# rlorenzo/facet

Measured on AMD Instinct MI355X. Metric: images/sec whole-node (TOPIQ+SAMP+CLIP+InsightFace ensemble), 1024² batch, higher is better.
Workload: dtype f32

## Files before the change

### facet_amd/_lib.py

```python
import ctypes as C
import importlib.util
import os
import sys
import threading

import numpy as np

_HERE = os.path.dirname(os.path.abspath(__file__))
LIB_PATH = os.environ.get("FACET_AMD_LIB") or os.path.join(_HERE, "libfacet_engine.so")

FE_MODEL_TOPIQ, FE_MODEL_CLIP, FE_MODEL_SAMP, FE_MODEL_U2NETP, FE_MODEL_AESTHETIC, FE_MODEL_VLM = range(6)
FE_RECORD_FLOATS = 789
FE_GRAPH_FACE_DET, FE_GRAPH_FACE_LMK, FE_GRAPH_FACE_REC = 0, 1, 2
FE_FACE_FLOATS = 739
FE_STATS_DOUBLES = 264
FILTERS = {"lanczos": 1, "bilinear": 2, "bicubic": 3}
FE_PRECISION_RES32 = 16
FE_PRECISION_SPLIT3 = 32
PRECISION = {"f32": 0, "fp32": 0, "float32": 0, "bf16": 1, "bfloat16": 1, "f16": 2, "fp16": 2, "float16": 2, "half": 2,
             "bf16+r32": 1 | FE_PRECISION_RES32, "f16+r32": 2 | FE_PRECISION_RES32, "f16x3": 2 | FE_PRECISION_RES32 | FE_PRECISION_SPLIT3}
PRECISION_NAME = {0: "f32", 1: "bf16", 2: "f16", 1 | FE_PRECISION_RES32: "bf16+r32", 2 | FE_PRECISION_RES32: "f16+r32",
                  2 | FE_PRECISION_RES32 | FE_PRECISION_SPLIT3: "f16x3"}
ACT = {"none": 0, None: 0, "relu": 1, "gelu": 2, "sigmoid": 3, "softplus": 5, "quickgelu": 6}
ELEM = {"f32": 0, "bf16": 1, "f16": 2}
# ... 45 lines not shown
    "fe_profile_get": (C.c_int, [C.c_void_p, C.c_int, C.c_char_p, C.c_int, C.POINTER(C.c_double),
                                 C.POINTER(C.c_double), _f32p]),
    "fe_flops_reset": (C.c_int, [C.c_void_p]),
    "fe_flops_get": (C.c_int, [C.c_void_p, C.POINTER(C.c_double)]),
    "fe_flops_get_executed": (C.c_int, [C.c_void_p, C.POINTER(C.c_double)]),
    "fe_flops_get_half": (C.c_int, [C.c_void_p, C.POINTER(C.c_double)]),
    "fe_weights_begin": (C.c_int, [C.c_void_p, C.c_int]),
    "fe_weights_set": (C.c_int, [C.c_void_p, C.c_int, C.c_char_p, _f32p, _i64p, C.c_int]),
    "fe_weights_commit": (C.c_int, [C.c_void_p, C.c_int]),
    "fe_model_unload": (C.c_int, [C.c_void_p, C.c_int]),
    "fe_model_loaded": (C.c_int, [C.c_void_p, C.c_int]),
    "fe_op_conv2d": (C.c_int, [C.c_void_p, _f32p, C.c_int, C.c_int, C.c_int, C.c_int, _f32p, C.c_int, C.c_int,
                               C.c_int, _f32p, _f32p, _f32p, C.c_int, C.c_int, C.c_int, C.c_int, C.c_int, _f32p]),
    "fe_op_gate_rowpool": (C.c_int, [C.c_void_p, _f32p, C.c_int, C.c_int, C.c_int, C.c_int, C.c_int, _f32p, _f32p, C.c_int, _f32p, C.c_int,
                                     C.c_int, C.c_int, C.c_int, _f32p, C.POINTER(C.c_int)]),
    "fe_op_topiq_gate64": (C.c_int, [C.c_void_p, _f32p, C.c_int, C.c_int, C.c_int, _f32p, _f32p, _f32p, _f32p, _f32p, C.c_float,
                                     _f32p, _f32p, C.c_int, C.c_int, _f32p]),
    "fe_op_conv3x3_c64": (C.c_int, [C.c_void_p, _f32p, C.c_int, C.c_int, C.c_int, _f32p, _f32p, _f32p, C.c_int, _f32p, _f32p, _f32p,
                                    _f32p, _f32p]),
    "fe_op_maxpool2d": (C.c_int, [C.c_void_p, _f32p, C.c_int, C.c_int, C.c_int, C.c_int, C.c_int, C.c_int,
                                  C.c_int, C.c_int, _f32p]),
    "fe_op_bilinear": (C.c_int, [C.c_void_p, _f32p, C.c_int, C.c_int, C.c_int, C.c_int, C.c_int, C.c_int, _f32p]),
    "fe_op_adaptive_avgpool": (C.c_int, [C.c_void_p, _f32p, C.c_int, C.c_int, C.c_int, C.c_int, C.c_int, C.c_int,
                                         _f32p]),
    "fe_op_layernorm": (C.c_int, [C.c_void_p, _f32p, C.c_int, C.c_int, _f32p, _f32p, C.c_float, _f32p]),
    "fe_op_plane": (C.c_int, [C.c_void_p, C.c_int, C.c_int, _f32p] + [C.c_int] * 14 + [C.c_float, C.c_float, _f32p]),
    "fe_op_rowpass": (C.c_int, [C.c_void_p, C.c_int, C.c_int, C.c_int, _f32p] + [C.c_int] * 6 + [_f32p, _f32p, C.c_int, C.c_int, C.c_float, C.c_float, _f32p]),
    "fe_op_gemm_skinny": (C.c_int, [C.c_void_p, C.c_int, C.c_int, C.c_int, _f32p, C.c_int, C.c_int, C.c_int, _f32p, C.c_int, C.c_int, _f32p, _f32p, C.c_int,
                                    C.c_int, C.c_float, _f32p]),
    "fe_op_attention": (C.c_int, [C.c_void_p, _f32p, _f32p, _f32p, _f32p, C.c_int, C.c_int, C.c_int, C.c_int, C.c_int, C.c_int, _f32p]),
# ... 389 lines not shown
        xr, xp = _f32(xr)
        weight, wp = _f32(weight)
        cout = weight.shape[0]
        assert weight.shape == (cout, cin)
        bp = None
        if bias is not None:
            bias, bp = _f32(bias)
        gate, gp = _f32(gate)
        assert gate.shape == (n, h, w)
        y = np.empty((n, th, tw, cout), np.float32)
        routed = C.c_int(0)
        self._ck(self.lib.fe_op_gate_rowpool(self.h, xp, n, h, w, cin, ldx, wp, bp, cout, gp, ACT[act], th, tw, int(bool(fused)),
                                             y.ctypes.data_as(_f32p), C.byref(routed)))
        return np.ascontiguousarray(y.transpose(0, 3, 1, 2)), bool(routed.value)

    def topiq_gate64(self, x, w0, b0, w2, b2, w4, b4, wx, bx, wblk_act="gelu", gate_act="gelu"):
        x, xp = _f32(x)
        n, c, h, w = x.shape
        assert c == 64
        arrs = [_f32(a) for a in (w0, b0, w2, b2, w4, wx, bx)]
        y = np.empty((n, 64, h // 16, w // 16), np.float32)
        self._ck(self.lib.fe_op_topiq_gate64(self.h, xp, n, h, w, arrs[0][1], arrs[1][1], arrs[2][1], arrs[3][1], arrs[4][1], C.c_float(float(b4)),
                                             arrs[5][1], arrs[6][1], ACT[wblk_act], ACT[gate_act], y.ctypes.data_as(_f32p)))
        return y

    def conv3x3_c64(self, x, w2, scale2=None, shift2=None, act2="relu", w3=None, scale3=None, shift3=None, res=None):
        x, xp = _f32(x)
        n, c, h, w = x.shape
        assert c == 64
        keep = [_f32(a) if a is not None else (None, None) for a in (w2, scale2, shift2, w3, scale3, shift3, res)]
# ... 1136 lines not shown
```

### facet_amd/csrc/capi_ops.hip

```cpp
#include "capi_internal.h"
#include "fp8_core.h"

template <class E>
static E* hook_up(Ctx& C, const float* src, size_t n, int off = 0) {
  if (!src) return nullptr;
  if constexpr (std::is_same_v<E, float>) {
    float* d = C.arena.array<float>(n + off) + off;
    FE_HIP(hipMemcpyAsync(d, src, n * sizeof(float), hipMemcpyHostToDevice, C.stream));
    return d;
  } else {
    const float* d32 = upload(C, src, n);
    E* d = C.arena.array<E>(n + off) + off;
    launch_convert(d32, d, n, C.stream);
    return d;
  }
}
template <class E>
static E* hook_filled(Ctx& C, size_t n, float fill, int off = 0) {
  const std::vector<float> v(n, fill);
  E* d = hook_up<E>(C, v.data(), n, off);
  FE_HIP(hipStreamSynchronize(C.stream));
  return d;
}
template <class E>
// ... 116 lines not shown
    W.shape = {cout, cin}; W.data.assign(weight, weight + (size_t)cout * cin);
    if (bias) { B.shape = {cout}; B.data.assign(bias, bias + cout); }
    ConvW cw = build_linear_rows(dw, W, bias ? &B : nullptr, 0, cout);
    FE_CHECK(cw.CinPad <= ldx, "fe_op_gate_rowpool: ldx below the packed channel count %d", cw.CinPad);
    Tensor xt = C.arena.tensor(n, h, w, ldx);
    FE_HIP(hipMemcpyAsync(xt.p, x, xt.numel() * sizeof(float), hipMemcpyHostToDevice, C.stream));
    Tensor gt = C.arena.tensor(n, h, w, 1);
    FE_HIP(hipMemcpyAsync(gt.p, gate, gt.numel() * sizeof(float), hipMemcpyHostToDevice, C.stream));
    ConvOpts og; og.act = act; og.gate = &gt;
    int took = 0;
    Tensor pooled = topiq_gate_pool(C, cw, xt.slice(0, cw.CinPad), og, th, tw, fused != 0, &took);
    FE_CHECK(pooled.h == th && pooled.w == tw && pooled.ld == cout, "fe_op_gate_rowpool: unexpected result shape");
    FE_HIP(hipMemcpyAsync(y, pooled.p, pooled.numel() * sizeof(float), hipMemcpyDeviceToHost, C.stream));
    FE_HIP(hipStreamSynchronize(C.stream));
    if (routed) *routed = took;
  });
}

int fe_op_topiq_gate64(fe_ctx* ctx, const float* x, int n, int h, int w, const float* w0, const float* b0, const float* w2, const float* b2,
                       const float* w4, float b4, const float* wx, const float* bx, int wblk_act, int gate_act, float* y) {
  return fe_api(ctx, [&] {
    Ctx& C = ctx->c;
    FE_CHECK(x && w0 && b0 && w2 && b2 && w4 && wx && bx && y && n > 0 && h > 0 && w > 0 && h % 16 == 0 && w % 16 == 0, "bad gate64 arguments");
    FE_CHECK(C.precision == PREC_BF16 || C.precision == PREC_F16, "fe_op_topiq_gate64: the fused gate exists for the 2-byte element types only");
    C.arena.reset();
    DeviceWeights dw;
    dw.prec = C.precision;
    GatedConvW g;
    build_gate64_fragments(dw, g, w0, b0, w2, b2, w4, b4, wx, bx);
    auto run = [&](auto* tag) {
// ... 570 lines not shown
```

### facet_amd/csrc/conv_bf16_kernel.h

```cpp
#pragma once
#include "fe_common.h"
#include <cstdlib>

namespace fe {

typedef float h_f32x16 __attribute__((ext_vector_type(16)));
typedef float h_v4f __attribute__((ext_vector_type(4)));
typedef __attribute__((address_space(3))) void* h_lptr_t;

union H8 {
  h_v4f f;
  uint4 u;
};

template <class E>
__device__ __forceinline__ void h_unpack8(const uint4 u, float v[8]) {
  const E* tag = nullptr;
  fe_unpack2(tag, u.x, v[0], v[1]); fe_unpack2(tag, u.y, v[2], v[3]);
  fe_unpack2(tag, u.z, v[4], v[5]); fe_unpack2(tag, u.w, v[6], v[7]);
}


typedef unsigned h_v2u __attribute__((ext_vector_type(2)));
typedef unsigned h_v4u __attribute__((ext_vector_type(4)));
// ... 632 lines not shown
      const bool cok = col < p.Cout;
      const float sc = (cok && p.scale) ? p.scale[col] : 1.f;
      const float sf = (cok && p.shift) ? p.shift[col] : 0.f;
  #pragma unroll
      for (int i = 0; i < TM; ++i) {
  #pragma unroll
        for (int e = 0; e < 16; ++e) {
          const int row = wm * TM * 32 + i * 32 + (e & 3) + 8 * (e >> 2) + 4 * h;
          const int m = m0 + row;
          if (cok && m < p.M) {
            float v = acc[i][j][e] * sc + sf;
            float rs_ = p.res ? (float)p.res[(size_t)m * p.ldr + col] : 0.f;
            if constexpr (S32) { if (p.res32) rs_ = p.res32[(size_t)m * p.ldr32 + col]; }
            if (!p.res_after_act) v += rs_;
            if constexpr (MODE == 2) v = v > 0.f ? v : v * p.slope[col];
            else v = fe_apply_act(v, p.act);
            if (p.res_after_act) v += rs_;
            if (p.gate) v *= (float)p.gate[(size_t)m * p.ldg + (p.gate_c1 ? 0 : col)];
            if constexpr (S32) {
              if (p.y) stf(&p.y[(size_t)m * p.ldy + col], v);
              if (p.y32) p.y32[(size_t)m * p.ldy32 + col] = v;
            } else {
              stf(&p.y[(size_t)m * p.ldy + col], v);
            }
          }
        }
      }
    }
  
    return;
// ... 47 lines not shown
```

### facet_amd/csrc/engine.h

```cpp
#pragma once
#include "fe_common.h"
#include "../../include/facet_engine.h"
#include <memory>
#include <tuple>

namespace fe {

struct HostTensor {
  std::vector<float> data;
  std::vector<int64_t> shape;
  size_t numel() const { size_t n = 1; for (auto d : shape) n *= (size_t)d; return n; }
};

class WeightStore {
 public:
  void clear() { t_.clear(); }
  void set(const std::string& name, const float* data, const int64_t* shape, int ndim);
  bool has(const std::string& name) const { return t_.count(name) != 0; }
  const HostTensor& get(const std::string& name) const;
  size_t size() const { return t_.size(); }
 private:
  std::map<std::string, HostTensor> t_;
};

// ... 66 lines not shown
  void* wv_h = nullptr;
  float* bv = nullptr;
  ConvW out;
  int d = 0, heads = 0;
};
MHAW build_mha(DeviceWeights& dw, const WeightStore& ws, const std::string& prefix, int heads);
template <class T, class RT>
void mha_forward(Ctx& c, const MHAW& m, const T* q_in, int ldq, const T* kv_in, int ldkv, int B, int Lq,
                 int Lk, const RT* res, int ldr, RT* y, int ldy, bool causal = false);
void linear_forward(Ctx& c, const ConvW& w, const float* x, int ldx, int M, float* y, int ldy, int act,
                    const float* res = nullptr, int ldr = 0);
void linear_forward(Ctx& c, const ConvW& w, const bf16* x, int ldx, int M, bf16* y, int ldy, int act,
                    const bf16* res = nullptr, int ldr = 0);
void linear_forward(Ctx& c, const ConvW& w, const f16* x, int ldx, int M, f16* y, int ldy, int act,
                    const f16* res = nullptr, int ldr = 0);
void linear_forward_s32(Ctx& c, const ConvW& w, const bf16* x, int ldx, int M, float* y, int ldy, int act, const float* res = nullptr, int ldr = 0);
void linear_forward_s32(Ctx& c, const ConvW& w, const f16* x, int ldx, int M, float* y, int ldy, int act, const float* res = nullptr, int ldr = 0);
void linear_forward_res(Ctx& c, const ConvW& w, const float* x, int ldx, int M, float* y, int ldy, int act, const float* res, int ldr);
void linear_forward_res(Ctx& c, const ConvW& w, const bf16* x, int ldx, int M, bf16* y, int ldy, int act, const bf16* res, int ldr);
void linear_forward_res(Ctx& c, const ConvW& w, const f16* x, int ldx, int M, f16* y, int ldy, int act, const f16* res, int ldr);
void linear_forward_res(Ctx& c, const ConvW& w, const bf16* x, int ldx, int M, float* y, int ldy, int act, const float* res, int ldr);
void linear_forward_res(Ctx& c, const ConvW& w, const f16* x, int ldx, int M, float* y, int ldy, int act, const float* res, int ldr);
void linear_forward_f32(Ctx& c, const ConvW& w, const float* x, int ldx, int M, float* y, int ldy, int act);
void linear_forward_f32(Ctx& c, const ConvW& w, const bf16* x, int ldx, int M, float* y, int ldy, int act);
void linear_forward_f32(Ctx& c, const ConvW& w, const f16* x, int ldx, int M, float* y, int ldy, int act);
void linear_forward_xf32(Ctx& c, const ConvW& w, int prec, const float* x, int ldx, int M, float* y, int ldy, int act);
template <class T>
inline TensorT<T> mat_view(const T* p, int rows, int cols, int ld) {
  TensorT<T> t; t.p = const_cast<T*>(p); t.n = 1; t.h = 1; t.w = rows; t.c = cols; t.ld = ld; return t;
}

void conv_forward(Ctx& c, const ConvW& w, const Tensor& x, const Tensor& y, const ConvOpts& o);
void conv_forward(Ctx& c, const ConvW& w, const TensorH& x, const TensorH& y, const ConvOptsT<bf16>& o);
void conv_forward(Ctx& c, const ConvW& w, const TensorF16& x, const TensorF16& y, const ConvOptsT<f16>& o);
bool conv_rowpool_ok(const Ctx& c, const ConvW& w, const Tensor& x, const ConvOpts& o, int kw);
template <class T>
TensorT<T> conv_new(Ctx& c, const ConvW& w, const TensorT<T>& x, const ConvOptsT<T>& o);
template <class T>
TensorT<T> first_conv(Ctx& c, const ConvW& w, const Tensor& x, const ConvOpts& o);
inline int conv_out_dim(int in, int k, int s, int p, int d) { return (in + 2 * p - d * (k - 1) - 1) / s + 1; }

struct ResBlock {
  ConvW c1, c2, c3, down;
  bool has_down = false, bottleneck = true;
  int stride = 1;
  void* frag2 = nullptr;
  void* frag3 = nullptr;
};
float* build_n16_weights(DeviceWeights& dw, const float* W, int cin);
void launch_conv3x3_n16_f32(const Tensor& x, const Tensor& y, const float* wt, const float* scale, const float* shift, int act, hipStream_t s);
// ... 312 lines not shown
```

### facet_amd/csrc/engine.hip

```cpp
#include "engine.h"
#include "onnx_graph.h"
#include "wino64_maps.h"
#include <algorithm>
#include <cmath>
#include <cstdlib>

namespace fe {

void WeightStore::set(const std::string& name, const float* data, const int64_t* shape, int ndim) {
  HostTensor h;
  h.shape.assign(shape, shape + ndim);
  h.data.assign(data, data + h.numel());
  t_[name] = std::move(h);
}
const HostTensor& WeightStore::get(const std::string& name) const {
  auto it = t_.find(name);
  if (it == t_.end()) throw Error("missing weight tensor '" + name + "'");
  return it->second;
}

float* DeviceWeights::upload(const std::vector<float>& v) {
  void* p = nullptr;
  const size_t b = v.size() * sizeof(float);
  FE_HIP(hipMalloc(&p, b ? b : 16));
// ... 210 lines not shown
  l.eps = eps;
  return l;
}

bool conv_rowpool_ok(const Ctx& c, const ConvW& w, const Tensor& x, const ConvOpts& o, int kw) {
  auto al16 = [](const void* ptr) { return ((uintptr_t)ptr & 15) == 0; };
  if (kw != 2 && kw != 4 && kw != 8 && kw != 16) return false;
  if (w.KH != 1 || w.KW != 1 || o.sh != 1 || o.sw != 1 || o.ph != 0 || o.pw != 0 || o.res || !o.gate || o.act == ACT_PRELU) return false;
  if (x.w % kw != 0 || x.c != w.CinPad || w.CinPad % 32 != 0 || w.Kp != w.CinPad || w.Cout <= 32 || w.Cout % 4 != 0) return false;
  if (c.force_variant != 0 || getenv("FE_NO_DMA")) return false;
  if (!al16(x.p) || x.ld % 4 != 0 || (w.scale && !al16(w.scale)) || (w.shift && !al16(w.shift))) return false;
  if (o.gate && o.gate->c != 1 && (o.gate->ld % 4 != 0 || !al16(o.gate->p))) return false;
  const unsigned long long img = (unsigned long long)x.h * x.w * (unsigned long long)(x.ld > w.Cout ? x.ld : w.Cout) * 4;
  const unsigned long long wspan = (unsigned long long)w.Cout * w.Kp * 4;
  return img < 0xF0000000ull && wspan < 0xFFFFFF00ull && x.pixels() < (1ull << 31);
}

void conv_forward(Ctx& c, const ConvW& w, const Tensor& x, const Tensor& y, const ConvOpts& o) {
  FE_CHECK(x.c == w.CinPad, "conv: input channels %d != packed Cin %d", x.c, w.CinPad);
  FE_CHECK(y.c == w.Cout && y.n == x.n, "conv: output view mismatch (c=%d Cout=%d)", y.c, w.Cout);
  ConvParams p{};
  p.x = x.p; p.ldx = x.ld;
  p.w = w.w; p.scale = w.scale; p.shift = w.shift; p.slope = w.slope;
  FE_CHECK(o.act != ACT_PRELU || w.slope, "conv: PReLU without slopes");
  if (o.res) {
    FE_CHECK(o.res->c == y.c && o.res->pixels() == y.pixels(), "conv: residual shape mismatch");
    p.res = o.res->p; p.ldr = o.res->ld;
  }
  if (o.gate) {
    FE_CHECK(o.gate->pixels() == y.pixels() && (o.gate->c == 1 || o.gate->c == y.c), "conv: gate shape mismatch");
// ... 66 lines not shown
        FE_HIP(hipEventSynchronize(e1));
        float ms = 0.f;
        FE_HIP(hipEventElapsedTime(&ms, e0, e1));
        (void)hipEventDestroy(e0); (void)hipEventDestroy(e1);
        char nm[128];
        snprintf(nm, sizeof nm, "wino3x3 M=%d K=%d N=%d", p.M, p.K, p.Cout);
        c.timings.push_back({nm, 2.0 * p.M * (double)(9 * w.Cin) * p.Cout, 0.0, ms});
      }
      c.arena.rewind(mark);
      c.flops_accum += 2.0 * p.M * (double)(w.KH * w.KW * w.Cin) * (w.CoutAlg ? w.CoutAlg : p.Cout);
      c.flops_saved += 2.0 * p.M * (double)(9 * w.Cin) * (w.CoutAlg ? w.CoutAlg : p.Cout) - 2.0 * (double)planes * (double)tiles * w.CinPad * w.Cout;
      return;
    }
  }
  static const bool no_wino64 = getenv("FE_NO_WINO64") != nullptr;
  if (w.wino64 && !no_wino64 && p.variant == 0 && (o.act == ACT_NONE || o.act == ACT_RELU || o.act == ACT_PRELU) && o.sh == 1 && o.sw == 1 && o.ph == 1 && o.pw == 1 && o.dh == 1 && o.dw == 1 && !o.gate && y.h == x.h &&
      y.w == x.w && (((uintptr_t)x.p | (uintptr_t)y.p | (uintptr_t)(o.res ? o.res->p : nullptr)) & 15) == 0 && x.ld % 4 == 0 && y.ld % 4 == 0 &&
      (!o.res || o.res->ld % 4 == 0) && (unsigned long long)x.h * x.w * x.ld * 4ull < 0xF0000000ull) {
    hipEvent_t e0 = nullptr, e1 = nullptr;
    if (c.profile) {
      FE_HIP(hipEventCreate(&e0)); FE_HIP(hipEventCreate(&e1));
      FE_HIP(hipEventRecord(e0, c.stream));
    }
    launch_wino64(x, y, w.wino64, w.scale, w.shift, w.slope, o.act, o.res, o.res_after_act, c.stream);
    const double direct = 2.0 * p.M * (double)(9 * w.Cin) * (w.CoutAlg ? w.CoutAlg : p.Cout);
    if (c.profile) {
      FE_HIP(hipEventRecord(e1, c.stream));
      FE_HIP(hipEventSynchronize(e1));
      float ms = 0.f;
      FE_HIP(hipEventElapsedTime(&ms, e0, e1));
      (void)hipEventDestroy(e0); (void)hipEventDestroy(e1);
      char nm[128];
      snprintf(nm, sizeof nm, "wino64 3x3 M=%d K=%d N=%d", p.M, p.K, p.Cout);
      const double bytes = 4.0 * ((double)x.pixels() * x.c + (double)y.pixels() * y.c * (o.res ? 2 : 1) + (double)w64::U_FLOATS);
      c.timings.push_back({nm, direct, bytes, ms});
    }
    const double tiles = (double)x.n * ((x.h + 1) / 2) * ((x.w + 1) / 2);
    c.flops_accum += direct;
    c.flops_saved += direct - 2.0 * 16.0 * tiles * 64.0 * w.Cout;
    return;
  }
  static const bool no_splitk = getenv("FE_NO_SPLITK") != nullptr;
  static const int splitk_min = getenv("FE_SPLITK_MIN") ? atoi(getenv("FE_SPLITK_MIN")) : 2048;
  if (!no_splitk && w.KH == 1 && w.KW == 1 && o.sh == 1 && o.sw == 1 && o.ph == 0 && o.pw == 0 && !o.gate && p.variant == 0 && p.M <= 256 &&
      w.CinPad >= splitk_min && w.K == w.CinPad && (size_t)((p.M + 127) / 128) * ((w.Cout + 63) / 64) < 64 &&
      (o.act == ACT_NONE || o.act == ACT_RELU || o.act == ACT_PRELU)) {
    int splits = 0;
    for (int s = 64; s >= 2; --s)
      if (w.CinPad % s == 0 && (w.CinPad / s) % 32 == 0 && w.CinPad / s >= 256) { splits = s; break; }
    const size_t part_bytes = (size_t)splits * p.M * w.Cout * sizeof(float);
    if (splits && c.arena.mark() + part_bytes + 1024 <= c.arena.capacity()) {
      const size_t mark = c.arena.mark();
      float* part = (float*)c.arena.alloc(part_bytes);
      const int Ks = w.CinPad / splits;
      hipEvent_t e0 = nullptr, e1 = nullptr;
      if (c.profile) {
// ... 441 lines not shown
static const bf16* mha_wv(const MHAW& m, const bf16*) {
  FE_CHECK(m.wv_h && m.q.hprec == PREC_BF16, "mha(bf16): model was not committed under bf16 precision");
  return (const bf16*)m.wv_h;
}
static const f16* mha_wv(const MHAW& m, const f16*) {
  FE_CHECK(m.wv_h && m.q.hprec == PREC_F16, "mha(f16): model was not committed under f16 precision");
  return (const f16*)m.wv_h;
}

void linear_forward_res(Ctx& c, const ConvW& w, const float* x, int ldx, int M, float* y, int ldy, int act, const float* res, int ldr) { linear_forward(c, w, x, ldx, M, y, ldy, act, res, ldr); }
void linear_forward_res(Ctx& c, const ConvW& w, const bf16* x, int ldx, int M, bf16* y, int ldy, int act, const bf16* res, int ldr) { linear_forward(c, w, x, ldx, M, y, ldy, act, res, ldr); }
void linear_forward_res(Ctx& c, const ConvW& w, const f16* x, int ldx, int M, f16* y, int ldy, int act, const f16* res, int ldr) { linear_forward(c, w, x, ldx, M, y, ldy, act, res, ldr); }
void linear_forward_res(Ctx& c, const ConvW& w, const bf16* x, int ldx, int M, float* y, int ldy, int act, const float* res, int ldr) { linear_forward_s32(c, w, x, ldx, M, y, ldy, act, res, ldr); }
void linear_forward_res(Ctx& c, const ConvW& w, const f16* x, int ldx, int M, float* y, int ldy, int act, const float* res, int ldr) { linear_forward_s32(c, w, x, ldx, M, y, ldy, act, res, ldr); }

template <class T, class RT>
void mha_forward(Ctx& c, const MHAW& m, const T* q_in, int ldq, const T* kv_in, int ldkv, int B, int Lq, int Lk,
                 const RT* res, int ldr, RT* y, int ldy, bool causal) {
  constexpr bool half = sizeof(T) == 2;
  const int d = m.d, H = m.heads, hd = d / H;
  const int Lp = (Lk + 31) / 32 * 32;
  const size_t mark = c.arena.mark();
  T* Q = c.arena.array<T>((size_t)B * Lq * d);
  T* K = c.arena.array<T>((size_t)B * Lk * d);
  T* Vt = c.arena.array<T>((size_t)B * d * Lp);
  static const bool no_flash = getenv("FE_NO_FLASH") != nullptr;
  const bool flash = (hd == 64) && (!no_flash || half);
  FE_CHECK(flash || !causal, "causal attention needs the fused kernel (head_dim 64)");
  FE_CHECK(flash || !half, "attention(bf16) needs head_dim 64");
  T* S = flash ? nullptr : c.arena.array<T>((size_t)B * H * Lq * Lp);
  T* O = c.arena.array<T>((size_t)B * Lq * d);
  linear_forward(c, m.q, q_in, ldq, B * Lq, Q, d, ACT_NONE);
  linear_forward(c, m.k, kv_in, ldkv, B * Lk, K, d, ACT_NONE);
  if (Lp != Lk) FE_HIP(hipMemsetAsync(Vt, 0, (size_t)B * d * Lp * sizeof(T), c.stream));
  {
    ConvParamsT<T> p{};
    p.x = mha_wv(m, q_in); p.ldx = d; p.w = kv_in; p.ldw = ldkv; p.y = Vt; p.ldy = Lp;
    p.M = d; p.K = d; p.Cout = Lk;
    p.batch = B; p.nb1 = 1; p.ws2 = (long long)Lk * ldkv; p.ys2 = (long long)d * Lp;
    p.pad_store = half ? 1 : 0;
    raw_gemm(c, p, 2.0 * B * d * (double)d * Lk);
  }
  if (flash) {
    launch_attention(Q, d, K, d, Vt, Lp, m.bv, O, d, B, H, Lq, Lk, d, causal ? 1 : 0, c.stream);
    c.flops_accum += 4.0 * B * H * (double)Lq * Lk * hd;
    if (half) c.flops_half += 4.0 * B * H * (double)Lq * Lk * hd;
  } else if constexpr (!half) {
    {
// ... 32 lines not shown
```

### facet_amd/csrc/fe_common.h

```cpp
#pragma once
#include <hip/hip_runtime.h>
#include "fe_check.h"
#include <cstdint>
#include <cstdio>
#include <atomic>
#include <cstring>
#include <map>
#include <mutex>
#include <stdexcept>
#include <string>
#include <utility>
#include <vector>

namespace fe {


#define FE_HIP(expr)                                                                      \
  do {                                                                                    \
    hipError_t _e = (expr);                                                               \
    if (_e != hipSuccess) {                                                               \
      char _b[512];                                                                       \
      snprintf(_b, sizeof _b, "%s:%d: %s -> %s", __FILE__, __LINE__, #expr,               \
               hipGetErrorString(_e));                                                    \
      throw fe::Error(_b);                                                                \
// ... 1 lines not shown
  } while (0)

inline void ensure_dynamic_lds(const void* kernel, size_t bytes, std::atomic<uint64_t>& done) {
  int dev = 0;
  FE_HIP(hipGetDevice(&dev));
  const uint64_t bit = 1ull << (dev & 63);
  if (done.load(std::memory_order_acquire) & bit) return;
  FE_HIP(hipFuncSetAttribute(kernel, hipFuncAttributeMaxDynamicSharedMemorySize, (int)bytes));
  done.fetch_or(bit, std::memory_order_release);
}

enum Act : int { ACT_NONE = 0, ACT_RELU = 1, ACT_GELU = 2, ACT_SIGMOID = 3, ACT_PRELU = 4, ACT_SOFTPLUS = 5, ACT_QUICKGELU = 6 };

__device__ __forceinline__ float fe_apply_act(float v, int act) {
  if (act == ACT_RELU) return v > 0.f ? v : 0.f;
  if (act == ACT_GELU) return 0.5f * v * (1.f + erff(v * 0.70710678118654752440f));
  if (act == ACT_SIGMOID) return 1.f / (1.f + __expf(-v));
  if (act == ACT_SOFTPLUS) return v > 20.f ? v : log1pf(expf(v));
  if (act == ACT_QUICKGELU) return v / (1.f + __expf(-1.702f * v));
  return v;
}

__device__ __forceinline__ float fe_rcp_fast(float x) { return __builtin_amdgcn_rcpf(x); }

__device__ __forceinline__ float fe_erf_as(float x) {
  const float ax = fabsf(x);
  const float t = fe_rcp_fast(1.0f + 0.3275911f * ax);
  const float poly = t * (0.254829592f + t * (-0.284496736f + t * (1.421413741f + t * (-1.453152027f + t * 1.061405429f))));
  const float r = 1.0f - poly * __expf(-ax * ax);
  return copysignf(r, x);
}
// ... 368 lines not shown
```

### facet_amd/csrc/kernels_conv_dma.hip

```cpp
#include "fe_common.h"
#include <cstdlib>

namespace fe {

typedef float f32x16 __attribute__((ext_vector_type(16)));
typedef float v4f __attribute__((ext_vector_type(4)));

__device__ __forceinline__ float apply_act_d(float v, int act) { return fe_apply_act(v, act); }

typedef const __attribute__((address_space(1))) void* gptr_t;
typedef __attribute__((address_space(3))) void* lptr_t;

template <int WGM, int WGN, int TM, int TN, int MODE = 0, bool ONE_TAP = false>
__global__ __launch_bounds__(256, (MODE == 1 ? 4 : (TM * TN >= 8 ? 2 : (TM * TN >= 4 ? 3 : 4)))) void conv_dma_kernel(ConvParams p, const int ntiles) {
  constexpr int BM = WGM * TM * 32, BN = WGN * TN * 32, BK = 16;
  constexpr int AI = (BM + 63) / 64, BI = (BN + 63) / 64;
  constexpr int SLAB = (BM + BN) * BK;
  static_assert(WGM * WGN == 4, "4 waves");
  extern __shared__ __attribute__((aligned(16))) float smem[];

  if (p.batch > 1) {
    const int b = blockIdx.y, bo = b / p.nb1, bi = b - bo * p.nb1;
    p.x += bo * p.xs2 + bi * p.xs1;
    p.w += bo * p.ws2 + bi * p.ws1;
// ... 549 lines not shown
      const float rf[4] = {ru.x, ru.y, ru.z, ru.w}, gf[4] = {gu.x, gu.y, gu.z, gu.w};
  #pragma unroll
      for (int e = 0; e < 4; ++e) {
        float x = v[e] * sc[e] + sf[e];
        if (p.res && !p.res_after_act) x += rf[e];
        v[e] = x;
      }
      if constexpr (MODE == 2) {
  #pragma unroll
        for (int e = 0; e < 4; ++e) v[e] = v[e] > 0.f ? v[e] : v[e] * sl[e];
      } else if (act == ACT_RELU) {
  #pragma unroll
        for (int e = 0; e < 4; ++e) v[e] = v[e] > 0.f ? v[e] : 0.f;
      } else if (act == ACT_GELU) {
  #pragma unroll
        for (int e = 0; e < 4; ++e) v[e] = 0.5f * v[e] * (1.f + erff(v[e] * 0.70710678118654752440f));
      } else if (act == ACT_SIGMOID) {
  #pragma unroll
        for (int e = 0; e < 4; ++e) v[e] = 1.f / (1.f + __expf(-v[e]));
      } else if (act == ACT_SOFTPLUS) {
  #pragma unroll 1
        for (int e = 0; e < 4; ++e) v[e] = v[e] > 20.f ? v[e] : log1pf(expf(v[e]));
      }
  #pragma unroll
      for (int e = 0; e < 4; ++e) {
        float x = v[e];
        if (p.res && p.res_after_act) x += rf[e];
        if (p.gate) x *= gf[e];
        v[e] = x;
      }
      if (cok && m < p.M) {
// ... 115 lines not shown
```

### facet_amd/csrc/kernels_wino64.hip

```cpp
#include "fe_common.h"
#include "wino64_maps.h"

namespace fe {

struct W64Params {
  const float* x; int ldx, cin;
  int N, H, W;
  float* y; int ldy, cout;
  const float* U;
  const float *scale, *shift, *slope;
  const float* res; int ldr;
  int res_after_act;
  int bx, by, nblocks;
};

constexpr int W64_PATCH_FLOATS = w64::CHUNK_UNITS * 2;

template <int A>
__global__ __launch_bounds__(256, 1) __attribute__((amdgpu_waves_per_eu(1, 1))) void wino64_kernel(const W64Params p) {
  using namespace w64;
  __shared__ __attribute__((aligned(16))) float sP[2 * W64_PATCH_FLOATS];
  const int t = threadIdx.x, lane = t & 63, wave = __builtin_amdgcn_readfirstlane(t >> 6);
  const int tg = wave & 1, half = wave >> 1;
  const int tl = lane & 31, kk = lane >> 5;
// ... 145 lines not shown
          q.x = fe_apply_act(q.x, act); q.y = fe_apply_act(q.y, act); q.z = fe_apply_act(q.z, act); q.w = fe_apply_act(q.w, act);
        }
        if (p.res && p.res_after_act) { q.x += r.x; q.y += r.y; q.z += r.z; q.w += r.w; }
        *reinterpret_cast<float4*>(p.y + pix[i] * p.ldy + cb) = q;
      }
    }
  }
}

void launch_wino64(const Tensor& x, const Tensor& y, const float* U, const float* scale, const float* shift, const float* slope, int act,
                   const Tensor* res, int res_after_act, hipStream_t s) {
  FE_CHECK(x.c > 0 && x.c <= 64 && x.c % 4 == 0 && y.c > 0 && y.c <= 64 && y.c % 4 == 0 && y.n == x.n && y.h == x.h && y.w == x.w, "wino64: %dx%dx%d -> %dx%dx%d", x.h,
           x.w, x.c, y.h, y.w, y.c);
  FE_CHECK(x.ld % 4 == 0 && y.ld % 4 == 0 && (((uintptr_t)x.p | (uintptr_t)y.p | (uintptr_t)U) & 15) == 0, "wino64: operands must be 16-byte aligned");
  FE_CHECK(!res || (res->ld % 4 == 0 && ((uintptr_t)res->p & 15) == 0 && res->c == y.c && res->pixels() == y.pixels()), "wino64: residual view");
  FE_CHECK(act == ACT_NONE || act == ACT_RELU || (act == ACT_PRELU && slope), "wino64: activation %d (PReLU needs slopes)", act);
  FE_CHECK((unsigned long long)x.h * x.w * x.ld * 4ull < 0xF0000000ull, "wino64: one image must stay below 4 GiB (32-bit buffer offsets)");
  W64Params p{};
  p.x = x.p; p.ldx = x.ld; p.cin = x.c; p.N = x.n; p.H = x.h; p.W = x.w;
  p.y = y.p; p.ldy = y.ld; p.cout = y.c;
  p.U = U; p.scale = scale; p.shift = shift; p.slope = slope;
  p.res = res ? res->p : nullptr; p.ldr = res ? res->ld : 0;
  p.res_after_act = res_after_act;
  p.bx = (x.w + w64::BLOCK - 1) / w64::BLOCK; p.by = (x.h + w64::BLOCK - 1) / w64::BLOCK;
  const long long nb = (long long)x.n * p.bx * p.by;
  FE_CHECK(nb < (1ll << 30), "wino64: too many blocks");
  p.nblocks = (int)nb;
  const int grid = p.nblocks < 256 ? p.nblocks : 256;
  if (act == ACT_NONE) hipLaunchKernelGGL(wino64_kernel<ACT_NONE>, dim3(grid), dim3(256), 0, s, p);
  else if (act == ACT_RELU) hipLaunchKernelGGL(wino64_kernel<ACT_RELU>, dim3(grid), dim3(256), 0, s, p);
  else hipLaunchKernelGGL(wino64_kernel<ACT_PRELU>, dim3(grid), dim3(256), 0, s, p);
  FE_HIP(hipGetLastError());
}

}
```

### facet_amd/csrc/model_topiq.hip

```cpp
#include "engine.h"
#include <algorithm>
#include <cmath>

namespace fe {

static EncLayerW build_enc(DeviceWeights& dw, const WeightStore& ws, const std::string& p, int heads) {
  EncLayerW e;
  e.attn = build_mha(dw, ws, p + ".self_attn", heads);
  e.lin1 = build_linear(dw, ws, p + ".linear1", true);
  e.lin2 = build_linear(dw, ws, p + ".linear2", true);
  e.n1 = build_ln(dw, ws, p + ".norm1");
  e.n2 = build_ln(dw, ws, p + ".norm2");
  return e;
}

static DecLayerW build_dec(DeviceWeights& dw, const WeightStore& ws, const std::string& p, int heads) {
  DecLayerW d;
  d.cross = build_mha(dw, ws, p + ".multihead_attn", heads);
  d.lin1 = build_linear(dw, ws, p + ".linear1", true);
  d.lin2 = build_linear(dw, ws, p + ".linear2", true);
  d.n1 = build_ln(dw, ws, p + ".norm1");
  d.n2 = build_ln(dw, ws, p + ".norm2");
  d.n3 = build_ln(dw, ws, p + ".norm3");
  return d;
// ... 110 lines not shown
template <class T>
static void ln(Ctx& c, const LayerNormW& l, const T* x, T* y, int rows) {
  launch_layernorm(x, l.d, y, l.d, l.g, l.b, rows, l.d, l.eps, c.stream);
}

template <class T>
static void enc_forward(Ctx& c, const EncLayerW& e, T* x, T* y, int B, int L) {
  const int d = e.n1.d, rows = B * L, ff = e.lin1.Cout;
  const size_t mark = c.arena.mark();
  T* n = c.arena.array<T>((size_t)rows * d);
  T* a = c.arena.array<T>((size_t)rows * d);
  T* hbuf = c.arena.array<T>((size_t)rows * ff);
  ln(c, e.n1, x, n, rows);
  mha_forward<T>(c, e.attn, n, d, n, d, B, L, L, x, d, a, d);
  ln(c, e.n2, a, n, rows);
  linear_forward(c, e.lin1, n, d, rows, hbuf, ff, ACT_GELU);
  linear_forward(c, e.lin2, hbuf, ff, rows, y, d, ACT_NONE, a, d);
  c.arena.rewind(mark);
}

template <class T>
static void dec_forward(Ctx& c, const DecLayerW& w, T* tgt, const T* memory, int B, int Lq, int Lk) {
  const int d = w.n1.d, ff = w.lin1.Cout;
  const size_t mark = c.arena.mark();
  T* mem = c.arena.array<T>((size_t)B * Lk * d);
  T* t2 = c.arena.array<T>((size_t)B * Lq * d);
  T* a = c.arena.array<T>((size_t)B * Lq * d);
  T* hbuf = c.arena.array<T>((size_t)B * Lq * ff);
  ln(c, w.n2, memory, mem, B * Lk);
  ln(c, w.n1, (const T*)tgt, t2, B * Lq);
  mha_forward<T>(c, w.cross, t2, d, mem, d, B, Lq, Lk, tgt, d, a, d);
  ln(c, w.n3, (const T*)a, t2, B * Lq);
  linear_forward(c, w.lin1, t2, d, B * Lq, hbuf, ff, ACT_GELU);
  linear_forward(c, w.lin2, hbuf, ff, B * Lq, tgt, d, ACT_NONE, a, d);
  c.arena.rewind(mark);
}

Tensor topiq_gate_pool(Ctx& c, const ConvW& split_x1, const Tensor& f, const ConvOpts& og, int th, int tw, bool rowpool, int* fused) {
  if (fused) *fused = 0;
  const int kw = (tw > 0 && f.w % tw == 0) ? f.w / tw : 0;
  if (rowpool && f.h > th && f.w > tw && th > 0 && f.h % th == 0 && kw && conv_rowpool_ok(c, split_x1, f, og, kw)) {
    Tensor pooled = c.arena.tensor(f.n, th, tw, split_x1.Cout);
    const size_t mark = c.arena.mark();
    Tensor part = c.arena.tensor(f.n, f.h, tw, split_x1.Cout);
    Tensor shape = f;
    shape.p = nullptr; shape.c = split_x1.Cout; shape.ld = split_x1.Cout;
    ConvOpts o = og;
    o.pool_kw = kw; o.pool = &part;
// ... 65 lines not shown
        if (c.profile) { FE_HIP(hipEventCreate(&e0)); FE_HIP(hipEventCreate(&e1)); FE_HIP(hipEventRecord(e0, c.stream)); }
        launch_conv3x3_c64(wa, wb, (const TensorT<T>*)nullptr, g.w2_frag, nullptr, nullptr, g.w2.shift, nullptr, nullptr, m.wblk_act, c.stream);
        if (c.profile) {
          FE_HIP(hipEventRecord(e1, c.stream)); FE_HIP(hipEventSynchronize(e1));
          float ms = 0.f;
          FE_HIP(hipEventElapsedTime(&ms, e0, e1));
          (void)hipEventDestroy(e0); (void)hipEventDestroy(e1);
          char nm[128];
          snprintf(nm, sizeof nm, "%s halo-tiled conv3x3 64->64 M=%d", PrecOf<T>::value == PREC_F16 ? "f16" : "bf16", (int)wa.pixels());
          c.timings.push_back({nm, flops, 2.0 * (double)wa.pixels() * 128, ms});
        }
        c.flops_accum += flops; c.flops_half += flops;
        tiled = true;
      }
    }
    if (!tiled) wb = conv_new(c, g.w2, wa, o2);
    ConvOptsT<T> o4; o4.act = ACT_SIGMOID; o4.ph = o4.pw = 1;
    TensorT<T> wc = conv_new(c, g.w4, wb, o4);
    ConvOptsT<T> og; og.act = m.gate_act; og.gate = &wc;
    TensorT<T> gated;
    if constexpr (sizeof(T) == 4) {
      const bool no_rowpool = getenv("FE_NO_GATE_ROWPOOL") != nullptr;
      const bool large = (size_t)f.h * f.w * g.split_x1.Cout * sizeof(float) >= ((size_t)1 << 20);
      gated = topiq_gate_pool(c, g.split_x1, f, og, th, tw, !no_rowpool && large);
    } else {
      gated = conv_new(c, g.split_x1, f, og);
      if (gated.h > th && gated.w > tw) {
        TensorT<T> pooled = c.arena.tensor_t<T>(B, th, tw, gated.c);
        launch_adaptive_avgpool(gated, pooled, c.stream);
        gated = pooled;
// ... 32 lines not shown
```

### include/facet_engine.h

```cpp
#ifndef FACET_ENGINE_H
#define FACET_ENGINE_H

#include <stddef.h>
#include <stdint.h>

#ifdef __cplusplus
extern "C" {
#endif

typedef struct fe_ctx fe_ctx;

enum fe_status {
  FE_OK = 0,
  FE_ERR_INVALID = -1,
  FE_ERR_RUNTIME = -2,
  FE_ERR_NOT_LOADED = -3,
  FE_ERR_CAPACITY = -4
};

enum fe_model {
  FE_MODEL_TOPIQ = 0,
  FE_MODEL_CLIP = 1,
  FE_MODEL_SAMP = 2,
  FE_MODEL_U2NETP = 3,
// ... 69 lines not shown

int fe_weights_begin(fe_ctx* ctx, int model);
int fe_weights_set(fe_ctx* ctx, int model, const char* name, const float* data, const int64_t* shape, int ndim);
int fe_weights_commit(fe_ctx* ctx, int model);
int fe_model_unload(fe_ctx* ctx, int model);
int fe_model_loaded(fe_ctx* ctx, int model);

int fe_op_conv2d(fe_ctx* ctx, const float* x, int n, int c, int h, int w, const float* weight, int cout, int kh,
                 int kw, const float* scale, const float* shift, const float* res, int res_after_act, int stride,
                 int pad, int dil, int act, float* y);
int fe_op_topiq_gate64(fe_ctx* ctx, const float* x, int n, int h, int w, const float* w0, const float* b0, const float* w2,
                       const float* b2, const float* w4, float b4, const float* wx, const float* bx, int wblk_act,
                       int gate_act, float* y);
int fe_op_gate_rowpool(fe_ctx* ctx, const float* x, int n, int h, int w, int cin, int ldx, const float* weight, const float* bias, int cout,
                       const float* gate, int act, int th, int tw, int fused, float* y, int* routed);
int fe_op_conv3x3_c64(fe_ctx* ctx, const float* x, int n, int h, int w, const float* w2, const float* scale2,
                      const float* shift2, int act2, const float* w3, const float* scale3, const float* shift3,
                      const float* res, float* y);
int fe_op_maxpool2d(fe_ctx* ctx, const float* x, int n, int c, int h, int w, int k, int stride, int pad,
                    int ceil_mode, float* y);
int fe_op_bilinear(fe_ctx* ctx, const float* x, int n, int c, int h, int w, int ho, int wo, float* y);
int fe_op_adaptive_avgpool(fe_ctx* ctx, const float* x, int n, int c, int h, int w, int ho, int wo, float* y);
int fe_op_layernorm(fe_ctx* ctx, const float* x, int rows, int d, const float* g, const float* b, float eps, float* y);
#define FE_ELEM_F32 0
#define FE_ELEM_BF16 1
#define FE_ELEM_F16 2
int fe_op_plane(fe_ctx* ctx, int route, int elem, const float* x, int n, int c, int h, int w, int ctot_in, int c0_in, int ctot_out, int c0_out,
                int k, int stride, int pad, int ceil_mode, int ho, int wo, float poison, float fill, float* y);
int fe_op_rowpass(fe_ctx* ctx, int route, int elem_in, int elem_out, const float* x, int rows, int d, int ldx, int ldy, int off_x, int off_y,
                  const float* g, const float* b, int off_gb, int L, float eps, float fill, float* y);
// ... 196 lines not shown
```

Before: 243.6.

## Route TOPIQ head GELU 3x3 convs through Winograd and add fast erf

Factors the Winograd 3x3 (wino64) dispatch into a reusable helper and gives it a GELU epilogue, so the large TOPIQ head gating conv can use Winograd instead of direct convolution. It also swaps erff in GELU for a custom polynomial erf built on a hardware exp2, and splits token linears into 32-row chunks when sequence length is short. A test entry point for wino64 is added. The custom erf and the Winograd transform may shift numerics slightly, and the chunked linears add extra kernel launches.

Measured after the change: 247.6, median of 6. 1.02x the previous value.

```diff
diff --git a/facet_amd/_lib.py b/facet_amd/_lib.py
--- a/facet_amd/_lib.py
+++ b/facet_amd/_lib.py
@@ -83,6 +83,7 @@
                                C.c_int, _f32p, _f32p, _f32p, C.c_int, C.c_int, C.c_int, C.c_int, C.c_int, _f32p]),
     "fe_op_gate_rowpool": (C.c_int, [C.c_void_p, _f32p, C.c_int, C.c_int, C.c_int, C.c_int, C.c_int, _f32p, _f32p, C.c_int, _f32p, C.c_int,
                                      C.c_int, C.c_int, C.c_int, _f32p, C.POINTER(C.c_int)]),
+    "fe_op_wino64": (C.c_int, [C.c_void_p, _f32p, C.c_int, C.c_int, C.c_int, C.c_int, _f32p, C.c_int, _f32p, _f32p, _f32p, C.c_int, C.c_int, _f32p]),
     "fe_op_topiq_gate64": (C.c_int, [C.c_void_p, _f32p, C.c_int, C.c_int, C.c_int, _f32p, _f32p, _f32p, _f32p, _f32p, C.c_float,
                                      _f32p, _f32p, C.c_int, C.c_int, _f32p]),
     "fe_op_conv3x3_c64": (C.c_int, [C.c_void_p, _f32p, C.c_int, C.c_int, C.c_int, _f32p, _f32p, _f32p, C.c_int, _f32p, _f32p, _f32p,
@@ -502,6 +503,24 @@
                                              y.ctypes.data_as(_f32p), C.byref(routed)))
         return np.ascontiguousarray(y.transpose(0, 3, 1, 2)), bool(routed.value)
 
+    def wino64_conv(self, x, w, scale=None, shift=None, res=None, res_after_act=False, act=None):
+        x, xp = _f32(x)
+        w, wp = _f32(w)
+        n, c, h, ww = x.shape
+        cout = w.shape[0]
+        assert w.shape == (cout, c, 3, 3)
+        y = np.empty((n, cout, h, ww), np.float32)
+        sp = hp = rp = None
+        if scale is not None:
+            scale, sp = _f32(scale)
+        if shift is not None:
+            shift, hp = _f32(shift)
+        if res is not None:
+            res, rp = _f32(res)
+            assert res.shape == y.shape
+        self._ck(self.lib.fe_op_wino64(self.h, xp, n, c, h, ww, wp, cout, sp, hp, rp, int(res_after_act), ACT[act], y.ctypes.data_as(_f32p)))
+        return y
+
     def topiq_gate64(self, x, w0, b0, w2, b2, w4, b4, wx, bx, wblk_act="gelu", gate_act="gelu"):
         x, xp = _f32(x)
         n, c, h, w = x.shape
diff --git a/facet_amd/csrc/capi_ops.hip b/facet_amd/csrc/capi_ops.hip
--- a/facet_amd/csrc/capi_ops.hip
+++ b/facet_amd/csrc/capi_ops.hip
@@ -1,5 +1,6 @@
 #include "capi_internal.h"
 #include "fp8_core.h"
+#include "wino64_maps.h"
 
 template <class E>
 static E* hook_up(Ctx& C, const float* src, size_t n, int off = 0) {
@@ -154,6 +155,26 @@
     FE_HIP(hipMemcpyAsync(y, pooled.p, pooled.numel() * sizeof(float), hipMemcpyDeviceToHost, C.stream));
     FE_HIP(hipStreamSynchronize(C.stream));
     if (routed) *routed = took;
+  });
+}
+
+int fe_op_wino64(fe_ctx* ctx, const float* x, int n, int c, int h, int w, const float* weight, int cout, const float* scale, const float* shift,
+                 const float* res, int res_after_act, int act, float* y) {
+  return fe_api(ctx, [&] {
+    Ctx& C = ctx->c;
+    FE_CHECK(x && weight && y && n > 0 && h > 0 && w > 0 && c > 0 && c <= 64 && c % 4 == 0 && cout > 0 && cout <= 64 && cout % 4 == 0, "bad wino64 arguments");
+    FE_CHECK(C.precision == PREC_F32, "fe_op_wino64: fp32 contexts only");
+    C.arena.reset();
+    std::vector<float> U(w64::U_FLOATS);
+    w64::pack_u(weight, cout, c, U.data());
+    const float* dU = upload(C, U.data(), U.size());
+    const float *ds = upload(C, scale, (size_t)cout), *dh = upload(C, shift, (size_t)cout);
+    Tensor xt = upload_nchw(C, x, n, c, h, w, c);
+    Tensor rt;
+    if (res) rt = upload_nchw(C, res, n, cout, h, w, cout);
+    Tensor yt = C.arena.tensor(n, h, w, cout);
+    launch_wino64(xt, yt, dU, ds, dh, nullptr, act, res ? &rt : nullptr, res_after_act, C.stream);
+    download_nchw(C, yt, cout, y);
   });
 }
 
diff --git a/facet_amd/csrc/conv_bf16_kernel.h b/facet_amd/csrc/conv_bf16_kernel.h
--- a/facet_amd/csrc/conv_bf16_kernel.h
+++ b/facet_amd/csrc/conv_bf16_kernel.h
@@ -670,6 +670,7 @@
             if constexpr (S32) { if (p.res32) rs_ = p.res32[(size_t)m * p.ldr32 + col]; }
             if (!p.res_after_act) v += rs_;
             if constexpr (MODE == 2) v = v > 0.f ? v : v * p.slope[col];
+            else if (p.act == ACT_GELU) v = 0.5f * v * (1.f + erff(v * 0.70710678118654752440f));
             else v = fe_apply_act(v, p.act);
             if (p.res_after_act) v += rs_;
             if (p.gate) v *= (float)p.gate[(size_t)m * p.ldg + (p.gate_c1 ? 0 : col)];
diff --git a/facet_amd/csrc/engine.h b/facet_amd/csrc/engine.h
--- a/facet_amd/csrc/engine.h
+++ b/facet_amd/csrc/engine.h
@@ -104,6 +104,9 @@
                     const bf16* res = nullptr, int ldr = 0);
 void linear_forward(Ctx& c, const ConvW& w, const f16* x, int ldx, int M, f16* y, int ldy, int act,
                     const f16* res = nullptr, int ldr = 0);
+void linear_tokens(Ctx& c, const ConvW& w, const float* x, int ldx, int B, int L, float* y, int ldy, int act);
+template <class T>
+inline void linear_tokens(Ctx& c, const ConvW& w, const T* x, int ldx, int B, int L, T* y, int ldy, int act) { linear_forward(c, w, x, ldx, B * L, y, ldy, act); }
 void linear_forward_s32(Ctx& c, const ConvW& w, const bf16* x, int ldx, int M, float* y, int ldy, int act, const float* res = nullptr, int ldr = 0);
 void linear_forward_s32(Ctx& c, const ConvW& w, const f16* x, int ldx, int M, float* y, int ldy, int act, const float* res = nullptr, int ldr = 0);
 void linear_forward_res(Ctx& c, const ConvW& w, const float* x, int ldx, int M, float* y, int ldy, int act, const float* res, int ldr);
@@ -124,6 +127,7 @@
 void conv_forward(Ctx& c, const ConvW& w, const TensorH& x, const TensorH& y, const ConvOptsT<bf16>& o);
 void conv_forward(Ctx& c, const ConvW& w, const TensorF16& x, const TensorF16& y, const ConvOptsT<f16>& o);
 bool conv_rowpool_ok(const Ctx& c, const ConvW& w, const Tensor& x, const ConvOpts& o, int kw);
+bool conv_wino64(Ctx& c, const ConvW& w, const Tensor& x, const Tensor& y, const ConvOpts& o);
 template <class T>
 TensorT<T> conv_new(Ctx& c, const ConvW& w, const TensorT<T>& x, const ConvOptsT<T>& o);
 template <class T>
diff --git a/facet_amd/csrc/engine.hip b/facet_amd/csrc/engine.hip
--- a/facet_amd/csrc/engine.hip
+++ b/facet_amd/csrc/engine.hip
@@ -248,6 +248,37 @@
   const unsigned long long img = (unsigned long long)x.h * x.w * (unsigned long long)(x.ld > w.Cout ? x.ld : w.Cout) * 4;
   const unsigned long long wspan = (unsigned long long)w.Cout * w.Kp * 4;
   return img < 0xF0000000ull && wspan < 0xFFFFFF00ull && x.pixels() < (1ull << 31);
+}
+
+bool conv_wino64(Ctx& c, const ConvW& w, const Tensor& x, const Tensor& y, const ConvOpts& o) {
+  if (!(w.wino64 && c.force_variant == 0 && w.KH == 3 && w.KW == 3 && o.sh == 1 && o.sw == 1 && o.ph == 1 && o.pw == 1 && o.dh == 1 && o.dw == 1 && !o.gate && !o.pool_kw &&
+        x.c == w.CinPad && y.c == w.Cout && y.n == x.n && y.h == x.h && y.w == x.w &&
+        (((uintptr_t)x.p | (uintptr_t)y.p | (uintptr_t)(o.res ? o.res->p : nullptr)) & 15) == 0 && x.ld % 4 == 0 && y.ld % 4 == 0 &&
+        (!o.res || o.res->ld % 4 == 0) && (unsigned long long)x.h * x.w * x.ld * 4ull < 0xF0000000ull && y.pixels() < (1ull << 31)))
+    return false;
+  const int M = (int)y.pixels();
+  hipEvent_t e0 = nullptr, e1 = nullptr;
+  if (c.profile) {
+    FE_HIP(hipEventCreate(&e0)); FE_HIP(hipEventCreate(&e1));
+    FE_HIP(hipEventRecord(e0, c.stream));
+  }
+  launch_wino64(x, y, w.wino64, w.scale, w.shift, w.slope, o.act, o.res, o.res_after_act, c.stream);
+  const double direct = 2.0 * M * (double)(9 * w.Cin) * (w.CoutAlg ? w.CoutAlg : w.Cout);
+  if (c.profile) {
+    FE_HIP(hipEventRecord(e1, c.stream));
+    FE_HIP(hipEventSynchronize(e1));
+    float ms = 0.f;
+    FE_HIP(hipEventElapsedTime(&ms, e0, e1));
+    (void)hipEventDestroy(e0); (void)hipEventDestroy(e1);
+    char nm[128];
+    snprintf(nm, sizeof nm, "wino64 3x3 M=%d K=%d N=%d", M, w.K, w.Cout);
+    const double bytes = 4.0 * ((double)x.pixels() * x.c + (double)y.pixels() * y.c * (o.res ? 2 : 1) + (double)w64::U_FLOATS);
+    c.timings.push_back({nm, direct, bytes, ms});
+  }
+  const double tiles = (double)x.n * ((x.h + 1) / 2) * ((x.w + 1) / 2);
+  c.flops_accum += direct;
+  c.flops_saved += direct - 2.0 * 16.0 * tiles * 64.0 * w.Cout;
+  return true;
 }
 
 void conv_forward(Ctx& c, const ConvW& w, const Tensor& x, const Tensor& y, const ConvOpts& o) {
@@ -344,32 +375,7 @@
     }
   }
   static const bool no_wino64 = getenv("FE_NO_WINO64") != nullptr;
-  if (w.wino64 && !no_wino64 && p.variant == 0 && (o.act == ACT_NONE || o.act == ACT_RELU || o.act == ACT_PRELU) && o.sh == 1 && o.sw == 1 && o.ph == 1 && o.pw == 1 && o.dh == 1 && o.dw == 1 && !o.gate && y.h == x.h &&
-      y.w == x.w && (((uintptr_t)x.p | (uintptr_t)y.p | (uintptr_t)(o.res ? o.res->p : nullptr)) & 15) == 0 && x.ld % 4 == 0 && y.ld % 4 == 0 &&
-      (!o.res || o.res->ld % 4 == 0) && (unsigned long long)x.h * x.w * x.ld * 4ull < 0xF0000000ull) {
-    hipEvent_t e0 = nullptr, e1 = nullptr;
-    if (c.profile) {
-      FE_HIP(hipEventCreate(&e0)); FE_HIP(hipEventCreate(&e1));
-      FE_HIP(hipEventRecord(e0, c.stream));
-    }
-    launch_wino64(x, y, w.wino64, w.scale, w.shift, w.slope, o.act, o.res, o.res_after_act, c.stream);
-    const double direct = 2.0 * p.M * (double)(9 * w.Cin) * (w.CoutAlg ? w.CoutAlg : p.Cout);
-    if (c.profile) {
-      FE_HIP(hipEventRecord(e1, c.stream));
-      FE_HIP(hipEventSynchronize(e1));
-      float ms = 0.f;
-      FE_HIP(hipEventElapsedTime(&ms, e0, e1));
-      (void)hipEventDestroy(e0); (void)hipEventDestroy(e1);
-      char nm[128];
-      snprintf(nm, sizeof nm, "wino64 3x3 M=%d K=%d N=%d", p.M, p.K, p.Cout);
-      const double bytes = 4.0 * ((double)x.pixels() * x.c + (double)y.pixels() * y.c * (o.res ? 2 : 1) + (double)w64::U_FLOATS);
-      c.timings.push_back({nm, direct, bytes, ms});
-    }
-    const double tiles = (double)x.n * ((x.h + 1) / 2) * ((x.w + 1) / 2);
-    c.flops_accum += direct;
-    c.flops_saved += direct - 2.0 * 16.0 * tiles * 64.0 * w.Cout;
-    return;
-  }
+  if (!no_wino64 && (o.act == ACT_NONE || o.act == ACT_RELU || o.act == ACT_PRELU) && conv_wino64(c, w, x, y, o)) return;
   static const bool no_splitk = getenv("FE_NO_SPLITK") != nullptr;
   static const int splitk_min = getenv("FE_SPLITK_MIN") ? atoi(getenv("FE_SPLITK_MIN")) : 2048;
   if (!no_splitk && w.KH == 1 && w.KW == 1 && o.sh == 1 && o.sw == 1 && o.ph == 0 && o.pw == 0 && !o.gate && p.variant == 0 && p.M <= 256 &&
@@ -841,6 +847,12 @@
 void linear_forward_res(Ctx& c, const ConvW& w, const bf16* x, int ldx, int M, float* y, int ldy, int act, const float* res, int ldr) { linear_forward_s32(c, w, x, ldx, M, y, ldy, act, res, ldr); }
 void linear_forward_res(Ctx& c, const ConvW& w, const f16* x, int ldx, int M, float* y, int ldy, int act, const float* res, int ldr) { linear_forward_s32(c, w, x, ldx, M, y, ldy, act, res, ldr); }
 
+void linear_tokens(Ctx& c, const ConvW& w, const float* x, int ldx, int B, int L, float* y, int ldy, int act) {
+  const int rows = B * L;
+  if (L > 32 || rows <= 32) { linear_forward(c, w, x, ldx, rows, y, ldy, act); return; }
+  for (int m0 = 0; m0 < rows; m0 += 32) linear_forward(c, w, x + (size_t)m0 * ldx, ldx, std::min(32, rows - m0), y + (size_t)m0 * ldy, ldy, act);
+}
+
 template <class T, class RT>
 void mha_forward(Ctx& c, const MHAW& m, const T* q_in, int ldq, const T* kv_in, int ldkv, int B, int Lq, int Lk,
                  const RT* res, int ldr, RT* y, int ldy, bool causal) {
@@ -857,8 +869,8 @@
   FE_CHECK(flash || !half, "attention(bf16) needs head_dim 64");
   T* S = flash ? nullptr : c.arena.array<T>((size_t)B * H * Lq * Lp);
   T* O = c.arena.array<T>((size_t)B * Lq * d);
-  linear_forward(c, m.q, q_in, ldq, B * Lq, Q, d, ACT_NONE);
-  linear_forward(c, m.k, kv_in, ldkv, B * Lk, K, d, ACT_NONE);
+  linear_tokens(c, m.q, q_in, ldq, B, Lq, Q, d, ACT_NONE);
+  linear_tokens(c, m.k, kv_in, ldkv, B, Lk, K, d, ACT_NONE);
   if (Lp != Lk) FE_HIP(hipMemsetAsync(Vt, 0, (size_t)B * d * Lp * sizeof(T), c.stream));
   {
     ConvParamsT<T> p{};
diff --git a/facet_amd/csrc/erf_core.h b/facet_amd/csrc/erf_core.h
--- /dev/null
+++ b/facet_amd/csrc/erf_core.h
@@ -0,0 +1,43 @@
+#pragma once
+#include <math.h>
+
+#ifdef __HIPCC__
+#include <hip/hip_runtime.h>
+#define FE_EHD __host__ __device__ __forceinline__
+#else
+#define FE_EHD inline
+#endif
+
+namespace fe {
+
+FE_EHD float fe_erf_exp2(float z) {
+#if defined(__HIP_DEVICE_COMPILE__)
+  return __builtin_amdgcn_exp2f(z);
+#else
+  return exp2f(z);
+#endif
+}
+
+FE_EHD float fe_erf(float x) {
+  const float t = fabsf(x), s = x * x;
+  float r = fmaf(0x1.222900p-16f, t, -0x1.91d2ccp-12f);
+  const float u = fmaf(0x1.fd1336p-09f, t, -0x1.8d6300p-06f);
+  r = fmaf(r, s, u);
+  r = fmaf(r, t, 0x1.b55cb0p-4f);
+  r = fmaf(r, t, 0x1.450aa0p-1f);
+  r = fmaf(r, t, 0x1.079d0cp-3f);
+  r = fmaf(r, t, t);
+  const float big = 1.0f - fe_erf_exp2(r * -1.44269504088896341f);
+  float p = -0x1.3a1a82p-11f;
+  p = fmaf(p, s, 0x1.473f48p-08f);
+  p = fmaf(p, s, -0x1.b68bd2p-06f);
+  p = fmaf(p, s, 0x1.ce1a46p-04f);
+  p = fmaf(p, s, -0x1.8126e0p-02f);
+  p = fmaf(p, s, 0x1.06eba6p-03f);
+  const float small = fmaf(p, t, t);
+  return copysignf(t > 0.921875f ? big : small, x);
+}
+
+FE_EHD float fe_gelu_erf(float v) { return 0.5f * v * (1.f + fe_erf(v * 0.70710678f)); }
+
+}
diff --git a/facet_amd/csrc/fe_common.h b/facet_amd/csrc/fe_common.h
--- a/facet_amd/csrc/fe_common.h
+++ b/facet_amd/csrc/fe_common.h
@@ -1,6 +1,7 @@
 #pragma once
 #include <hip/hip_runtime.h>
 #include "fe_check.h"
+#include "erf_core.h"
 #include <cstdint>
 #include <cstdio>
 #include <atomic>
@@ -39,7 +40,7 @@
 
 __device__ __forceinline__ float fe_apply_act(float v, int act) {
   if (act == ACT_RELU) return v > 0.f ? v : 0.f;
-  if (act == ACT_GELU) return 0.5f * v * (1.f + erff(v * 0.70710678118654752440f));
+  if (act == ACT_GELU) return fe_gelu_erf(v);
   if (act == ACT_SIGMOID) return 1.f / (1.f + __expf(-v));
   if (act == ACT_SOFTPLUS) return v > 20.f ? v : log1pf(expf(v));
   if (act == ACT_QUICKGELU) return v / (1.f + __expf(-1.702f * v));
diff --git a/facet_amd/csrc/kernels_conv_dma.hip b/facet_amd/csrc/kernels_conv_dma.hip
--- a/facet_amd/csrc/kernels_conv_dma.hip
+++ b/facet_amd/csrc/kernels_conv_dma.hip
@@ -587,7 +587,7 @@
         for (int e = 0; e < 4; ++e) v[e] = v[e] > 0.f ? v[e] : 0.f;
       } else if (act == ACT_GELU) {
   #pragma unroll
-        for (int e = 0; e < 4; ++e) v[e] = 0.5f * v[e] * (1.f + erff(v[e] * 0.70710678118654752440f));
+        for (int e = 0; e < 4; ++e) v[e] = fe_gelu_erf(v[e]);
       } else if (act == ACT_SIGMOID) {
   #pragma unroll
         for (int e = 0; e < 4; ++e) v[e] = 1.f / (1.f + __expf(-v[e]));
diff --git a/facet_amd/csrc/kernels_wino64.hip b/facet_amd/csrc/kernels_wino64.hip
--- a/facet_amd/csrc/kernels_wino64.hip
+++ b/facet_amd/csrc/kernels_wino64.hip
@@ -183,7 +183,7 @@
            x.w, x.c, y.h, y.w, y.c);
   FE_CHECK(x.ld % 4 == 0 && y.ld % 4 == 0 && (((uintptr_t)x.p | (uintptr_t)y.p | (uintptr_t)U) & 15) == 0, "wino64: operands must be 16-byte aligned");
   FE_CHECK(!res || (res->ld % 4 == 0 && ((uintptr_t)res->p & 15) == 0 && res->c == y.c && res->pixels() == y.pixels()), "wino64: residual view");
-  FE_CHECK(act == ACT_NONE || act == ACT_RELU || (act == ACT_PRELU && slope), "wino64: activation %d (PReLU needs slopes)", act);
+  FE_CHECK(act == ACT_NONE || act == ACT_RELU || act == ACT_GELU || (act == ACT_PRELU && slope), "wino64: activation %d (PReLU needs slopes)", act);
   FE_CHECK((unsigned long long)x.h * x.w * x.ld * 4ull < 0xF0000000ull, "wino64: one image must stay below 4 GiB (32-bit buffer offsets)");
   W64Params p{};
   p.x = x.p; p.ldx = x.ld; p.cin = x.c; p.N = x.n; p.H = x.h; p.W = x.w;
@@ -198,6 +198,7 @@
   const int grid = p.nblocks < 256 ? p.nblocks : 256;
   if (act == ACT_NONE) hipLaunchKernelGGL(wino64_kernel<ACT_NONE>, dim3(grid), dim3(256), 0, s, p);
   else if (act == ACT_RELU) hipLaunchKernelGGL(wino64_kernel<ACT_RELU>, dim3(grid), dim3(256), 0, s, p);
+  else if (act == ACT_GELU) hipLaunchKernelGGL(wino64_kernel<ACT_GELU>, dim3(grid), dim3(256), 0, s, p);
   else hipLaunchKernelGGL(wino64_kernel<ACT_PRELU>, dim3(grid), dim3(256), 0, s, p);
   FE_HIP(hipGetLastError());
 }
diff --git a/facet_amd/csrc/model_topiq.hip b/facet_amd/csrc/model_topiq.hip
--- a/facet_amd/csrc/model_topiq.hip
+++ b/facet_amd/csrc/model_topiq.hip
@@ -148,7 +148,7 @@
   ln(c, e.n1, x, n, rows);
   mha_forward<T>(c, e.attn, n, d, n, d, B, L, L, x, d, a, d);
   ln(c, e.n2, a, n, rows);
-  linear_forward(c, e.lin1, n, d, rows, hbuf, ff, ACT_GELU);
+  linear_tokens(c, e.lin1, n, d, B, L, hbuf, ff, ACT_GELU);
   linear_forward(c, e.lin2, hbuf, ff, rows, y, d, ACT_NONE, a, d);
   c.arena.rewind(mark);
 }
@@ -165,7 +165,7 @@
   ln(c, w.n1, (const T*)tgt, t2, B * Lq);
   mha_forward<T>(c, w.cross, t2, d, mem, d, B, Lq, Lk, tgt, d, a, d);
   ln(c, w.n3, (const T*)a, t2, B * Lq);
-  linear_forward(c, w.lin1, t2, d, B * Lq, hbuf, ff, ACT_GELU);
+  linear_tokens(c, w.lin1, t2, d, B, Lq, hbuf, ff, ACT_GELU);
   linear_forward(c, w.lin2, hbuf, ff, B * Lq, tgt, d, ACT_NONE, a, d);
   c.arena.rewind(mark);
 }
@@ -261,6 +261,15 @@
         tiled = true;
       }
     }
+    if constexpr (sizeof(T) == 4) {
+      const bool no_head_wino64 = getenv("FE_NO_HEAD_WINO64") != nullptr || getenv("FE_NO_WINO64") != nullptr;
+      const bool large = (size_t)wa.h * wa.w * g.w2.Cout * sizeof(float) >= ((size_t)1 << 20);
+      if (g.w2.wino64 && m.wblk_act == ACT_GELU && large && !no_head_wino64) {
+        wb = c.arena.tensor(wa.n, wa.h, wa.w, g.w2.Cout);
+        if (!conv_wino64(c, g.w2, wa, wb, o2)) conv_forward(c, g.w2, wa, wb, o2);
+        tiled = true;
+      }
+    }
     if (!tiled) wb = conv_new(c, g.w2, wa, o2);
     ConvOptsT<T> o4; o4.act = ACT_SIGMOID; o4.ph = o4.pw = 1;
     TensorT<T> wc = conv_new(c, g.w4, wb, o4);
diff --git a/include/facet_engine.h b/include/facet_engine.h
--- a/include/facet_engine.h
+++ b/include/facet_engine.h
@@ -107,6 +107,8 @@
                        int gate_act, float* y);
 int fe_op_gate_rowpool(fe_ctx* ctx, const float* x, int n, int h, int w, int cin, int ldx, const float* weight, const float* bias, int cout,
                        const float* gate, int act, int th, int tw, int fused, float* y, int* routed);
+int fe_op_wino64(fe_ctx* ctx, const float* x, int n, int c, int h, int w, const float* weight, int cout, const float* scale, const float* shift,
+                 const float* res, int res_after_act, int act, float* y);
 int fe_op_conv3x3_c64(fe_ctx* ctx, const float* x, int n, int h, int w, const float* w2, const float* scale2,
                       const float* shift2, int act2, const float* w3, const float* scale3, const float* shift3,
                       const float* res, float* y);
```
